# JADGardner/RENI

Measured on AMD Instinct MI355X. Metric: directional-samples/sec (fwd+bwd), 128x256 equirect, ND=36 latent, higher is better.
Workload: dtype bf16

## Files before the change

reni_amd/csrc/reni_capi.inc:

```
#include <dlfcn.h>

#include <cmath>
#include <cstdarg>
#include <cstdio>
#include <cstdlib>
#include <atomic>
#include <cstring>
#include <mutex>
#include <new>
#include <string>
#include <vector>

#include "../../include/reni_hip.h"

struct reni_plan {
  reni_desc d;
  int F_in;
  int64_t n_params;
  int64_t n_first;
  unsigned p_off_w[reni::MAX_LAYERS + 2];
  unsigned p_off_b[reni::MAX_LAYERS + 2];
  int M_in, N_out;
  int64_t n_map_params;
  unsigned mw_off[reni::MAX_MAP_LAYERS + 1], mb_off[reni::MAX_MAP_LAYERS + 1];
// ... 115 lines not shown
  }
  if (l.nwg < 1) l.nwg = 1;
  size_t o = 0;
  for (int st = 0; st < 2; ++st) {
    const bool mine = st == stage;
    if (mine) l.o_idxc = o;
    o += al256((size_t)B * 8);
    if (mine) l.o_Zc = o;
    o += al256((size_t)B * p->d.ndims * 3 * 4);
    if (mine) l.o_A = o;
    o += al256((size_t)B * H * 8 * 4);
    if (mine) l.o_afrag = o;
    if (l.persist) o += al256((size_t)B * (H / 32) * 1024);
    if (mine) l.o_xconst = o;
    o += al256((size_t)B * p->F_in * 4);
  }
  size_t w = 0;
  for (int i = 1; i <= L; ++i) { l.fwd_off[i] = (unsigned)w; w += al1k((size_t)g.img_hid + g.bias_hid); }
  l.fwd_off[L + 1] = (unsigned)w; w += al1k((size_t)g.img_hf + g.bias_head);
  for (int i = 1; i <= L; ++i) { l.bwd_off[i] = (unsigned)w; w += al1k((size_t)g.img_hid); }
  l.bwd_off[L + 1] = (unsigned)w; w += al1k((size_t)g.img_hb);
  l.wimg_bytes = w;
  w += 8192;
  l.o_wimg = o; o += al256(w);
  l.o_skip = o; o += 256;
  l.o_img_loss = o; o += al256((size_t)B * 16 * 4);
  l.o_stats = o; o += al256((size_t)B * 16 * 4);
  if (backward) {
    l.stash_per_wg = (size_t)(L + 1) * g.stash_layer_bytes * ((l.persist && !l.pdw && !l.wide_train) ? 2 : 1);
    l.frag = (p->d.dtype == RENI_BF16 && H == 256 && L >= 1 && (film || (flags & RENI_NEED_DW))) ? 1 : 0;
    if (p->d.dtype == RENI_F32 && H == 256 && L >= 1 && !film && (flags & RENI_NEED_DW)) l.frag = 2;
    l.o_stash = o; o += al256(l.stash_per_wg * (l.frag ? (size_t)l.n_tiles : (size_t)l.nwg));
    l.dwp_per_wg = (flags & RENI_NEED_DW) ? (size_t)(p->n_params - p->n_first) : 0;
    l.pkmax = ((l.n_tiles + l.nwg - 1) / l.nwg + l.tpi - 1) / l.tpi + 1;
    const size_t run_slots = (film && l.persist && !l.wide_train) ? (size_t)l.pkmax : 1;
    l.o_dwp = o; o += al256(l.dwp_per_wg * 4 * l.nwg * run_slots);
    l.o_dA_part = o; if (!l.pdw) o += al256((size_t)l.n_tiles * H * 8 * 4);
    l.o_tflag = l.o_tlist = l.o_tcount = l.o_imgcos = o;
    if (!film && !(flags & RENI_NEED_DW)) {
      l.o_tflag = o; o += al256((size_t)l.n_tiles * 4);
      l.o_tlist = o; o += al256((size_t)2 * l.n_tiles * 4);
      l.o_tcount = o; o += 256;
      l.o_imgcos = o; o += al256((size_t)B * 4);
      l.o_pcnt = o; o += al256((size_t)l.n_tiles * 4);
      l.o_pscan = o; o += al256((size_t)(l.n_tiles + 1) * 4);
      l.o_nlive = o; o += al256((size_t)B * 4);
      l.o_plist = o; o += al256((size_t)B * P * 4);
    }
    l.o_loss_part = o; o += al256((size_t)l.n_tiles * 4 * 16 * 4);
    l.o_dA = o; o += al256((size_t)B * H * 8 * 4);
    l.o_dw1p = o; if (l.pdw && (flags & RENI_NEED_DW)) o += al256((size_t)2 * l.nwg * run_slots * ((size_t)H * H + H) * 4);
    l.o_g1 = o; if (l.pdw) o += al256((size_t)((l.n_tiles + l.nwg - 1) / l.nwg) * l.nwg * (H / 16) * 4096);
    l.o_pruns = o; if (l.pdw) o += al256((size_t)l.nwg * l.pkmax * (H * 8 + 16) * 4);
    l.o_prunimg = o; if (l.pdw) o += al256((size_t)l.nwg * l.pkmax * (film ? 3 : 1) * 4);
    l.rt_chunk = reni::RT_CHUNK;
    l.nch = (l.tpi + l.rt_chunk - 1) / l.rt_chunk;
    l.o_part2 = o; o += al256((size_t)B * l.nch * (H * 8 + 16) * 4);
    l.o_mcol = o; o += al256((size_t)B * p->F_in * 4);
    l.o_ucol = o; o += al256((size_t)B * p->d.ndims * 3 * 4);
    l.o_dfp = o; if (film && !l.persist) o += al256((size_t)l.n_tiles * L * 2 * H * 4);
    const bool can = p->d.dtype == RENI_BF16 && L >= 1;
    l.stream = can && (H == 128 || H == 256) && (!l.persist || l.wide_train) && (film || (flags & RENI_NEED_DW)) ? 1 : 0;
    l.o_dws = o;
    l.o_dfr = o;
    l.o_runimg = o;
    if (l.frag == 2) o += al256((size_t)L * l.n_tiles * g.stash_layer_bytes);
// ... 98 lines not shown
bool dw1_ring_plan_ok(const reni_plan* p, int64_t P) { return !p->dw1_old && p->d.conditioning != RENI_COND_FILM && P % 128 == 0; }
bool dw1_ring_call_ok(const reni::MainArgs& a) { return (((uintptr_t)a.D | (uintptr_t)(a.d_bstride * 4)) & 15) == 0; }
int dw1_slots(bool ring, int nwg) { return ring ? nwg : 2 * nwg; }
bool l0x_rows_ok(const float* base, long long s0, long long s1, long long s2) {
  if (((uintptr_t)base | (uintptr_t)(s0 * 4)) & 15) return false;
  if (s1 == 3 && s2 == 1) return true;
  return s1 == 1 && ((uintptr_t)(s2 * 4) & 15) == 0;
}
bool l0x_plan_ok(const reni_plan* p, const Layout& l, int64_t P, uint32_t flags) {
  const int L = p->d.hidden_layers;
  return l.pdw && !p->no_l0x && dw1_ring_plan_ok(p, P) && spec_head(flags & RENI_NEED_DW, p->d.last_layer_linear, p->d.output_activation) &&
         L >= 3 && (L & 1) == 1;
}
bool l0x_call_ok(const reni::MainArgs& a) {
  return dw1_ring_call_ok(a) && train_spec(a, false) && l0x_rows_ok(a.target, a.ts0, a.ts1, a.ts2) && l0x_rows_ok(a.weight, a.ws0, a.ws1, a.ws2);
}
bool side_stream_plan_ok(const reni_plan* p, const Layout& l) { return l.pdw && !p->no_side_stream; }

int launch_dw1(const reni::MainArgs& a, int nwg, bool ring, hipStream_t s, bool l0x = false) {
#ifdef RENI_TRACE_DW1
  constexpr int TRACE = 8192;
#else
  constexpr int TRACE = 0;
#endif
  if (l0x)
    return timed_launch(reni::k_reni_l0_ring<128>, nwg, reni::L0Ring::THREADS, reni::L0Ring::LDS_BYTES + TRACE, s, a, PROF_DW1);
  if (a.film != nullptr) return timed_launch(s, PROF_DW1, "k_reni_dw1 (FiLM)", [&] { return reni::launch_dw1_film(a, 2 * nwg, s); });
  if (ring)
    return timed_launch(reni::k_reni_dw1_ring<128>, nwg, reni::Dw1Ring::THREADS, reni::Dw1Ring::LDS_BYTES + TRACE, s, a, PROF_DW1);
  return timed_launch(reni::k_reni_dw1<128>, 2 * nwg, 256, 2 * reni::TS_BYTES + TRACE, s, a, PROF_DW1);
}

int reduce_partials(const float* part, size_t per_wg, int nslot, float* out, int lo, int hi, const int* valid, const reni::LayerScale& lsc,
                    hipStream_t s) {
  RENI_LAUNCH(reni::k_reduce_partials, dim3((unsigned)((hi - lo + 63) / 64)), dim3(256), 0, s, part, per_wg, nslot, out, lo, hi, valid, lsc);
  return RENI_OK;
}

struct SideStream { hipStream_t s; hipEvent_t ev[3]; bool ok; };
std::mutex g_side_mu;
SideStream* side_stream() {
  static SideStream tab[16];
  static std::mutex mu;
  int dev = 0;
  if (hipGetDevice(&dev) != hipSuccess || dev < 0 || dev >= 16) return nullptr;
  std::lock_guard<std::mutex> lk(mu);
  SideStream& t = tab[dev];
  if (!t.ok) {
    if (hipStreamCreateWithFlags(&t.s, hipStreamNonBlocking) != hipSuccess) return nullptr;
    for (int i = 0; i < 3; ++i)
      if (hipEventCreateWithFlags(&t.ev[i], hipEventDisableTiming) != hipSuccess) return nullptr;
    t.ok = true;
  }
  return &t;
}

int launch_main(const reni_plan* p, int mode, const reni::MainArgs& a, int nwg, hipStream_t s) {
  const int H = p->d.hidden_features;
  const bool film = p->d.conditioning == RENI_COND_FILM, f32 = p->d.dtype == RENI_F32;
  return timed_launch(s, mode == reni::MODE_FWD_BWD ? PROF_FWD_BWD : mode == reni::MODE_STATS ? PROF_STATS : PROF_FWD, "fused kernel", [&] {
    if (f32) return film ? reni::launch_film_f32(H, mode, a, nwg, s) : reni::launch_main_f32(H, mode, a, nwg, s);
    return film ? reni::launch_film_bf16(H, mode, a, nwg, s) : reni::launch_main_bf16(H, mode, a, nwg, s);
  });
}

struct DeviceGuard {
  int prev = -1;
// ... 214 lines not shown
  uint32_t* state;
};

constexpr int LOSS_DOUT = 2;
struct BwdCall {
  int64_t B = 0, P = 0;
  const float *Z = nullptr, *D = nullptr, *params = nullptr;
  int64_t dbs = 0;
  const float *target = nullptr, *weight = nullptr, *dout = nullptr;
  const int64_t *ts = nullptr, *wst = nullptr;
  int loss_kind = RENI_LOSS_MSE;
  float alpha = 0.f, beta = 0.f;
  uint32_t flags = 0;
  float *out = nullptr, *loss_terms = nullptr, *dZ = nullptr, *dparams = nullptr;
  void* ws = nullptr;
  size_t ws_bytes = 0;
  void* stream = nullptr;
  const FilmIO* fio = nullptr;
  const int64_t* idx = nullptr;
  int64_t n_rows = 0;
  const StepFuse* fuse = nullptr;
  const WeightLists* lists = nullptr;
};

struct BwdPath {
  bool staged;
  int stage;
  bool use_cos;
  bool sparse;
  bool compact;
  bool cos_const;
  bool dw1_ring;
  bool l0x;
  bool fork;
  bool early_rest;
  bool dp_early;
  bool fused_tail;
  bool fuse_on;
  bool fpers;
  bool red2;
  int n_rest;
  int n_l1;
  bool rp_in_tail;
  bool ev_rest_done;
  bool dp_early_done;
};

struct Bwd {
  const reni_plan* p;
  const BwdCall& c;
  GeoRt g; Layout l; reni::MainArgs a;
  char* ws;
  hipStream_t s, se;
  const float* Z;
  int stage_in;
  float *img_loss, *stats, *dA, *part2;
  ListDst ld;
  reni::LayerScale lsc;
  BwdPath path;
};

bool call_uses_cos(const BwdCall& c) { return c.loss_kind == RENI_LOSS_TEST && c.beta != 0.f; }

BwdPath bwd_path(const reni_plan* p, const Layout& l, const BwdCall& c, const reni::MainArgs& a, int stage_in) {
  BwdPath t{};
  const int H = p->d.hidden_features, L = p->d.hidden_layers;
  const bool need_dw = (c.flags & RENI_NEED_DW) != 0;
  t.staged = stage_in >= 0;
  t.stage = t.staged ? stage_in : 0;
  t.n_rest = (int)(p->n_params - p->n_first);
  t.n_l1 = H * H + H;
  t.use_cos = call_uses_cos(c);
  t.sparse = (c.flags & (RENI_WEIGHT_SPARSE | RENI_WEIGHT_COMPACT)) && !c.fio && !need_dw && c.loss_kind != LOSS_DOUT &&
             c.weight != nullptr && c.out == nullptr;
  t.compact = t.sparse && (c.flags & RENI_WEIGHT_COMPACT);
  t.cos_const = t.sparse && c.lists && (c.lists->flags & RENI_WEIGHT_COS_CONSTANT);
  t.dw1_ring = dw1_ring_plan_ok(p, c.P) && dw1_ring_call_ok(a);
  t.l0x = l0x_plan_ok(p, l, c.P, c.flags) && l0x_call_ok(a);
  t.fork = side_stream_plan_ok(p, l) && !t.l0x && (c.fio || l.n_tiles >= 8 * l.nwg);
  t.early_rest = l.pdw && !c.fio && need_dw && L >= 1 && t.n_rest > t.n_l1;
  t.dp_early = c.fuse && c.fuse->comm && c.fuse->overlap;
  t.fused_tail = l.pdw && !c.fio;
  t.fuse_on = c.fuse && !c.fuse->comm && t.fused_tail && need_dw && (c.flags & RENI_NEED_DZ) && L >= 1;
  t.fpers = l.persist && !l.wide_train;
  t.red2 = L > 0 && t.fpers && need_dw;
  return t;
}

int bwd_validate(Bwd& x) {
  const reni_plan* p = x.p; const BwdCall& c = x.c;
  if (const int rc = c.fio ? check_film(p, c.fio, true) : RENI_OK) return rc;
  if (!c.fio && p && p->d.conditioning != RENI_COND_CONCAT) return fail(RENI_EINVAL, "FiLM plan: use the reni_film_* entry points");
  if (const int rc = check_common(p, c.B, c.P, c.fio ? c.fio->A : c.Z, c.D, c.params, c.ws)) return rc;
  if ((c.flags & RENI_NEED_DW) && !c.dparams) return fail(RENI_EINVAL, "RENI_NEED_DW set but dparams is NULL");
  if (!c.fio && (c.flags & RENI_NEED_DZ) && !c.dZ) return fail(RENI_EINVAL, "RENI_NEED_DZ set but dZ is NULL");
  if (c.loss_kind == LOSS_DOUT) {
    if (!c.dout) return fail(RENI_EINVAL, "dout is NULL");
  } else {
    if (c.loss_kind != RENI_LOSS_MSE && c.loss_kind != RENI_LOSS_TEST) return fail(RENI_EINVAL, "unknown loss_kind %d", c.loss_kind);
    if (!c.target || !c.weight || !c.ts || !c.wst) return fail(RENI_EINVAL, "target/weight (and their strides) must be non-NULL");
    if (!c.loss_terms) return fail(RENI_EINVAL, "loss_terms is NULL");
  }
  if (!geo_for(p, &x.g)) return fail(RENI_EUNSUPPORTED, "hidden_features=%d unsupported", p->d.hidden_features);
  return RENI_OK;
}

int bwd_layout(Bwd& x) {
  const BwdCall& c = x.c;
  const bool staged = c.fuse && (*c.fuse->state & 1u);
  x.stage_in = staged ? (int)((*c.fuse->state >> 1) & 1u) : -1;
  x.l = make_layout(x.p, x.g, c.B, c.P, c.flags, true, true, staged ? x.stage_in : 0);
// ... 59 lines not shown
}

int bwd_stats_pass(Bwd& x) {
  const BwdCall& c = x.c; const Layout& l = x.l;
  if (!x.path.use_cos || x.path.cos_const) return RENI_OK;
  reni::MainArgs st = x.a;
  st.out = nullptr; st.loss_kind = 0;
  if (x.path.sparse) { st.tlist = x.a.tlist + l.n_tiles; st.tcount = x.a.tcount + 1; }
  if (const int rc = l.persist ? launch_train(x.p, st, l.nwg, x.s, true) : launch_main(x.p, reni::MODE_STATS, st, l.nwg, x.s)) return rc;
  RENI_LAUNCH(reni::k_stats_image, dim3((unsigned)c.B), dim3(256), 0, x.s, (const float*)x.a.loss_part, l.tpi, c.weight, (long long)c.wst[0],
                     (long long)c.wst[2], c.beta, x.img_loss, x.stats, (const int*)x.ld.imgcos);
  return RENI_OK;
}

struct SideJoin {
  SideStream* side = nullptr;
  hipStream_t s = nullptr;
  ~SideJoin() { if (side && hipEventRecord(side->ev[2], side->s) == hipSuccess) (void)hipStreamWaitEvent(s, side->ev[2], 0); }
};

int bwd_fork_dw1(Bwd& x, std::unique_lock<std::mutex>& side_lock, SideJoin& side_join) {
  const reni_plan* p = x.p; const BwdCall& c = x.c; const Layout& l = x.l; BwdPath& path = x.path; hipStream_t s = x.s;
  if (!l.pdw) return RENI_OK;
  SideStream* side = path.fork ? side_stream() : nullptr;
  if (side) {
    side_lock.lock();
    HIP_TRY(hipEventRecord(side->ev[0], s));
    HIP_TRY(hipStreamWaitEvent(side->s, side->ev[0], 0));
    x.se = side->s;
    side_join.side = side; side_join.s = s;
  }
  path.rp_in_tail = path.early_rest && !side && !g_ev_rest && !path.dp_early;
  if (path.early_rest && !path.rp_in_tail) {
    int rc = reduce_partials(x.a.dwp, l.dwp_per_wg, l.nwg, c.dparams + p->n_first, path.n_l1, path.n_rest, nullptr, x.lsc, s);
    if (rc) return rc;
    if (g_ev_rest) { HIP_TRY(hipEventRecord(g_ev_rest, s)); path.ev_rest_done = true; }
    if (path.dp_early) {
      SideStream* cs = side_stream();
      if (!cs) return fail(RENI_EHIP, "no communication stream");
      if (!side_lock.owns_lock()) side_lock.lock();
      HIP_TRY(hipEventRecord(cs->ev[1], s));
      HIP_TRY(hipStreamWaitEvent(cs->s, cs->ev[1], 0));
      rc = rccl_allreduce_inplace(c.fuse->comm, c.dparams + p->n_first + path.n_l1, (size_t)(path.n_rest - path.n_l1), cs->s);
      if (rc) return rc;
      if (!side_join.side) { side_join.side = cs; side_join.s = s; }
      path.dp_early_done = true;
    }
  }
  return launch_dw1(x.a, l.nwg, path.dw1_ring, s, path.l0x);
}

int bwd_dw_consumers(Bwd& x) {
  const Layout& l = x.l; const reni::MainArgs& a = x.a; hipStream_t s = x.s;
  const int H = x.p->d.hidden_features;
  if (l.frag == 2) {
    const int lds = 4 * ((reni::Geo<reni::PolF32, 256>::T_BYTES + 1023) & ~1023);
    if (const int rc = timed_launch(reni::k_dw_frag32<256>, l.nwg, 256, lds, s, a, PROF_DWS)) return rc;
  }
  if (l.wide_train && (x.c.flags & RENI_NEED_DW)) {
    if (const int rc = timed_launch(s, PROF_DWS, "k_wide_head_dw", [&] { return reni::launch_wide_head_dw(a, l.nwg, s); })) return rc;
  }
  if (l.stream) {
    static_assert(reni::Geo<reni::PolBF16, 256>::T_BYTES_AL == 36864 && reni::Geo<reni::PolBF16, 128>::T_BYTES_AL == 34816,
                  "stream record sizes (make_layout)");
    const bool film = x.c.fio != nullptr;
    void (*fn)(const reni::MainArgs) = nullptr;
    if (H == 256) fn = film ? reni::k_dw_frag<256, true> : reni::k_dw_frag<256, false>;
// ... 57 lines not shown
  const reni_plan* p = x.p; const BwdCall& c = x.c; const Layout& l = x.l; const BwdPath& path = x.path; const reni::MainArgs& a = x.a;
  hipStream_t s = x.s, se = x.se;
  const int H = p->d.hidden_features;
  const bool need_dw = (c.flags & RENI_NEED_DW) != 0;
  reni::TailArgs t;
  t.dA = x.dA; t.W0 = c.params; t.Z = x.Z; t.xconst = (const float*)(x.ws + l.o_xconst);
  t.mcol = (float*)(x.ws + l.o_mcol); t.ucol = (float*)(x.ws + l.o_ucol);
  t.dZ = c.dZ; t.dW0 = c.dparams; t.db0 = c.dparams ? c.dparams + (size_t)H * p->F_in : nullptr;
  t.alpha2 = (c.loss_kind == RENI_LOSS_TEST) ? c.alpha : 0.f;
  t.eq = p->d.equivariance; t.nd = p->d.ndims; t.F_in = p->F_in; t.H = H; t.B = (int)c.B;
  if (!path.fuse_on && need_dw && l.pdw && p->d.hidden_layers >= 1) {
    if (const int rc = reduce_partials(a.dw1p, (size_t)path.n_l1, dw1_slots(path.dw1_ring, l.nwg), c.dparams + p->n_first, 0, path.n_l1, nullptr, x.lsc, s)) return rc;
  }
  reni::TailFusedArgs f;
  memset(&f, 0, sizeof(f));
  f.t = t;
  f.img_loss = x.img_loss; f.stats = x.stats; f.P = (int)c.P; f.nz = (int)(c.B * p->d.ndims * 3); f.has_cos = path.use_cos ? 1 : 0;
  f.has_prior = (c.loss_kind == RENI_LOSS_TEST) ? 1 : 0; f.alpha = c.alpha; f.beta = c.beta;
  f.loss_terms = (c.loss_kind != LOSS_DOUT) ? c.loss_terms : nullptr;
  f.need_dz = (c.flags & RENI_NEED_DZ) ? 1 : 0;
  f.need_dw0 = need_dw ? 1 : 0;
  f.dw0_gx = (p->F_in + 1 + 255) / 256;
  f.idx_now = path.staged ? (const long long*)c.idx : nullptr;
  f.idx_staged = path.staged ? (const long long*)(x.ws + l.o_idxc) : nullptr;
  f.skip_flag = c.fuse ? (int*)(x.ws + l.o_skip) : nullptr;
  const unsigned nb = (unsigned)((f.need_dz ? c.B : 0) + 1 + (f.need_dw0 ? f.dw0_gx * H : 0));
  if (path.fused_tail) {
    f.pruns = a.pruns; f.prun_image = a.prun_image; f.nwg = l.nwg; f.kmax = l.pkmax; f.tpi = l.tpi; f.n_tiles = l.n_tiles;
    f.dA_out = x.dA;
    const unsigned ny = f.need_dz ? (unsigned)((p->F_in + 63) / 64) : 1u;
    unsigned gx = (unsigned)c.B;
    if (path.rp_in_tail) {
      f.rp_part = a.dwp; f.rp_per_wg = l.dwp_per_wg; f.rp_nwg = l.nwg; f.rp_out = c.dparams + p->n_first; f.rp_lo = path.n_l1; f.rp_n = path.n_rest; f.rp_ls = x.lsc;
      gx += ((unsigned)((path.n_rest - path.n_l1 + 63) / 64) + ny - 1) / ny;
    }
    RENI_LAUNCH(reni::k_tail_a, dim3(gx, ny), dim3(256), (size_t)reni::tail_a_lds_bytes(H), se, f);
  } else if (c.flags & RENI_NEED_DZ) {
    RENI_LAUNCH(reni::k_tail_m, dim3((unsigned)c.B, (unsigned)((p->F_in + 63) / 64)), dim3(256), 0, se, t);
  }
  RENI_LAUNCH(reni::k_tail_b, dim3(nb), dim3(256), 0, se, f);
  if (need_dw && !path.fused_tail && path.n_rest > 0) {
    if (const int rc = reduce_partials(a.dwp, l.dwp_per_wg, l.nwg, c.dparams + p->n_first, 0, path.n_rest, nullptr, x.lsc, s)) return rc;
  }
  if (g_ev_rest && !path.ev_rest_done) HIP_TRY(hipEventRecord(g_ev_rest, s));
  return RENI_OK;
}

int bwd_fused_step(Bwd& x, SideJoin& side_join) {
  const reni_plan* p = x.p; const BwdCall& c = x.c; const Layout& l = x.l; const BwdPath& path = x.path; hipStream_t s = x.s;
  const StepFuse& fu = *c.fuse;
  if (side_join.side) {
    HIP_TRY(hipEventRecord(side_join.side->ev[2], side_join.side->s));
    HIP_TRY(hipStreamWaitEvent(s, side_join.side->ev[2], 0));
    side_join.side = nullptr;
  }
  if (fu.comm) {
    const size_t n_early = path.dp_early_done ? (size_t)(path.n_rest - path.n_l1) : 0;
    EvPair ev;
    const bool timed = prof_begin(s, &ev, PROF_COMM);
    int rc = rccl_allreduce_max_i32(fu.comm, (int*)(x.ws + l.o_skip), 1, s);
    if (rc) return rc;
    rc = rccl_allreduce_inplace(fu.comm, c.dparams, (size_t)p->n_params - n_early, s);
    if (rc) return rc;
    if (timed) HIP_TRY(hipEventRecord(ev.b, s));
  }
  reni::Adam2Args ad;
  ad.p = fu.params; ad.g = c.dparams; ad.m = fu.m_dec; ad.v = fu.v_dec; ad.n = p->n_params;
// ... 914 lines not shown
```

reni_amd/csrc/reni_dev_common.inc:

```


DEV constexpr int rowmap(int r, int hi) { return (r & 3) + 8 * (r >> 2) + 4 * hi; }

struct PolF32 {
  static constexpr bool BF = false;
  static constexpr int FRAGB = 4;
  static constexpr int KF = 2;
  static constexpr int TS = 2;
  static constexpr int WPS = 1;
  static constexpr int HEAD_BWD_KS = 3;
  static constexpr int STASH_CH_PER_RB = 4;
  using Frag = float;
  static DEV f32x16 mfma(Frag a, Frag b, f32x16 c) {
    return __builtin_amdgcn_mfma_f32_32x32x2f32(a, b, c, 0, 0, 0);
  }
  static DEV void drain() {
    __builtin_amdgcn_sched_barrier(0);
    asm volatile("s_nop 15\n\ts_nop 3");
    __builtin_amdgcn_sched_barrier(0);
  }
};
struct PolBF16 {
  static constexpr bool BF = true;
  static constexpr int FRAGB = 16;
// ... 458 lines not shown
          } else {
            *p = first ? acc[m][r] : (*p + acc[m][r]);
          }
        } else if constexpr (KIND == DW_HEAD) {
          if (j < 3) {
            float* p = dst_w + (size_t)j * ldw + row;
            *p = first ? acc[m][r] : (*p + acc[m][r]);
          }
        } else {
          const float lo = __shfl_down(acc[m][r], 8, 64);
          if (j < 8) dst_w[(size_t)row * 8 + j] = acc[m][r] + ((j < 4) ? lo : 0.f);
        }
      }
    }
  }
  if constexpr (!DO_B) {
    return;
  } else if constexpr (KIND == DW_HIDDEN) {
    dbacc += __shfl_xor(dbacc, 32, 64);
    if (wave < NBR && wave < NBLK && hi == 0) {
      if (rscale != nullptr) dbacc *= rscale[32 * (wave % NBR) + j];
      float* p = dst_b + 32 * (wave % NBR) + j;
      *p = first ? dbacc : (*p + dbacc);
    }
  } else if constexpr (KIND == DW_HEAD) {
    dbacc += __shfl_xor(dbacc, 32, 64);
    if (wave == 0 && hi == 0 && j < 3) {
      float* p = dst_b + j;
      *p = first ? dbacc : (*p + dbacc);
    }
  }
}

struct FilmDw {
  const float* fl;
  float* fs;
  const float* W;
  const float* b;
  float* out;
  int do_w;
};

DEV float half_sum(float t) {
#pragma unroll
  for (int o = 16; o >= 1; o >>= 1) t += __shfl_xor(t, o, 64);
  return t;
}

template <class Pol, int H, int NBR, int NBC, int KIND, bool FILM = false>
DEV void dw_phase(char* TA, char* TB, const float (&rows)[NBR][16], const float (&cols)[NBC][16],
                  float* dst_w, float* dst_b, int ldw, bool first, int wave, int lane, int dbg = 0,
                  const FilmDw* fd = nullptr) {
  constexpr int MYB = (NBR * NBC + 3) / 4;
  constexpr int NBLK = NBR * NBC;
  constexpr int NROUND = 4 / Geo<Pol, H>::ROUND_WAVES;
  const int hi = lane >> 5, j = lane & 31;
  const int tid = wave * 64 + lane;
  if constexpr (MYB <= 4) {
    f32x16 acc[MYB];
    acc_zero<MYB>(acc);
    float dbacc = 0.f;
#pragma unroll 1
    for (int round = 0; round < NROUND; ++round) {
      __syncthreads();
      if (wave / Geo<Pol, H>::ROUND_WAVES == round && !(dbg & 4)) {
        t_write<Pol, H, NBR>(TA, rows, wave % Geo<Pol, H>::ROUND_WAVES, hi, j);
// ... 177 lines not shown
```

reni_amd/csrc/reni_dev_small.inc:

```

DEV void reduce_film_runs_body(const MainArgs& a, int H, int nruns, float* dfilm, const int bx, const int by) {
  const float* dfr = a.dfr;
  const int* run_image = a.run_image;
  const int L = a.L;
  const float* params = a.params;
  const unsigned n_first = a.n_first;
  const unsigned* p_off_b = a.p_off_b;
  const int b = bx, i = by * 256 + threadIdx.x;
  const bool live = i < L * H;
  const int l = live ? i / H : 0, f = i - l * H;
  __shared__ int vl[1024];
  __shared__ int nv;
  float s0 = 0.f, s1 = 0.f;
  for (int base = 0; base < nruns; base += 1024) {
    const int cnt = nruns - base < 1024 ? nruns - base : 1024;
    __syncthreads();
    if (threadIdx.x < 64) {
      int c = 0;
      for (int w0 = 0; w0 < cnt; w0 += 64) {
        const int w = w0 + (int)threadIdx.x;
        const bool ok = w < cnt && run_image[base + w] == b;
        const unsigned long long m = __ballot(ok);
        if (ok) vl[c + __popcll(m & ((1ull << threadIdx.x) - 1ull))] = base + w;
        c += __popcll(m);
// ... 388 lines not shown
  const int i = (int)blockIdx.x;
  if (i < a.n_prep && a.film_A != nullptr) afrag_from_A_body(a.film_A, a.film_afrag, a.film_scale, a.prep.H, a.film_B, i);
  else if (i < a.n_prep) prep_image_body(a.prep, i / a.prep_gy, i % a.prep_gy, smem);
  else pack_body<Pol>(ka, (i - a.n_prep) % a.pack_gx, (i - a.n_prep) / a.pack_gx, a.pack_gx);
}
template __global__ void k_prologue<PolF32>(const PrologueArgs, const PackArgs);
template __global__ void k_prologue<PolBF16>(const PrologueArgs, const PackArgs);

struct LayerScale { int n_hid, L; float c[MAX_LAYERS + 1]; };
DEV float layer_scale(const LayerScale& ls, int e) {
  int k = ls.n_hid > 0 ? e / ls.n_hid : 0;
  k = k < ls.L ? k : ls.L;
  return ls.c[k];
}
DEV void reduce_partials_body(const float* part, size_t per_wg, int nwg, float* dparams, int lo, int n, int blk, float (*red2)[64],
                              const LayerScale& ls) {
  const int lane = threadIdx.x & 63, grp = threadIdx.x >> 6;
  const int e = lo + blk * 64 + lane;
  float s[8];
#pragma unroll
  for (int q = 0; q < 8; ++q) s[q] = 0.f;
  if (e < n) {
    int q = grp;
    for (; q + 28 < nwg; q += 32) {
#pragma unroll
      for (int u = 0; u < 8; ++u) s[u] += part[(size_t)(q + 4 * u) * per_wg + e];
    }
    for (; q < nwg; q += 4) s[0] += part[(size_t)q * per_wg + e];
  }
  red2[grp][lane] = ((s[0] + s[1]) + (s[2] + s[3])) + ((s[4] + s[5]) + (s[6] + s[7]));
  __syncthreads();
  if (grp == 0 && e < n) dparams[e] = ((red2[0][lane] + red2[1][lane]) + (red2[2][lane] + red2[3][lane])) * layer_scale(ls, e);
}
DEV void reduce_partials_valid_body(const float* part, size_t per_wg, int nwg, float* dparams, int lo, int n, const int* valid, int blk) {
  __shared__ int vl[2048];
  __shared__ int nv;
  __shared__ float red[4][64];
  const int lane = threadIdx.x & 63, grp = threadIdx.x >> 6;
  const int e = lo + blk * 64 + lane;
  float s[8];
#pragma unroll
  for (int q = 0; q < 8; ++q) s[q] = 0.f;
  for (int base = 0; base < nwg; base += 2048) {
    const int cnt = nwg - base < 2048 ? nwg - base : 2048;
    __syncthreads();
    if (threadIdx.x < 64) {
      int c = 0;
      for (int w0 = 0; w0 < cnt; w0 += 64) {
        const int w = w0 + (int)threadIdx.x;
        const bool ok = w < cnt && valid[base + w] >= 0;
        const unsigned long long m = __ballot(ok);
        if (ok) vl[c + __popcll(m & ((1ull << threadIdx.x) - 1ull))] = base + w;
        c += __popcll(m);
      }
      if (threadIdx.x == 0) nv = c;
    }
    __syncthreads();
    if (e < n) {
      const int m = nv;
      int q = grp;
      for (; q + 28 < m; q += 32) {
#pragma unroll
        for (int u = 0; u < 8; ++u) s[u] += part[(size_t)vl[q + 4 * u] * per_wg + e];
      }
      for (; q < m; q += 4) s[0] += part[(size_t)vl[q] * per_wg + e];
    }
  }
  red[grp][lane] = ((s[0] + s[1]) + (s[2] + s[3])) + ((s[4] + s[5]) + (s[6] + s[7]));
  __syncthreads();
  if (grp == 0 && e < n) dparams[e] = (red[0][lane] + red[1][lane]) + (red[2][lane] + red[3][lane]);
}
__global__ void __launch_bounds__(256) k_reduce_partials(const float* part, size_t per_wg, int nwg,
                                                          float* dparams, int lo, int n, const int* valid, const LayerScale ls) {
  const int i = lo + blockIdx.x * 256 + threadIdx.x;
  if (valid != nullptr) {
    reduce_partials_valid_body(part, per_wg, nwg, dparams, lo, n, valid, (int)blockIdx.x);
    return;
  }
  (void)i;
  __shared__ float red2[4][64];
  reduce_partials_body(part, per_wg, nwg, dparams, lo, n, (int)blockIdx.x, red2, ls);
}

struct FilmReduce2 { int H, nruns, B, gy; float* dfilm; const float* part; size_t per_wg; int nslot; float* dparams; int n; const int* valid; };
__global__ void __launch_bounds__(256) k_film_reduce2(const MainArgs a, const FilmReduce2 r) {
  const int i = (int)blockIdx.x, nb1 = r.B * r.gy;
  if (i < nb1) reduce_film_runs_body(a, r.H, r.nruns, r.dfilm, i / r.gy, i % r.gy);
  else reduce_partials_valid_body(r.part, r.per_wg, r.nslot, r.dparams, 0, r.n, r.valid, i - nb1);
}

constexpr int RT_CHUNK = 4;
__global__ void __launch_bounds__(256) k_reduce_tiles_a(const float* dA_part, const float* loss_part,
                                                        int tiles_per_image, int H, float* part2, int have_dA, int chunk,
                                                        const int* tflag = nullptr) {
  const int b = blockIdx.x, ch = blockIdx.y, nch = gridDim.y;
  const int t0 = ch * chunk, t1 = min(t0 + chunk, tiles_per_image);
  float* out = part2 + ((size_t)b * nch + ch) * (H * 8 + 16);
  if (have_dA) {
    const int k = threadIdx.x & 7;
    constexpr int MAXQ = 8;
    const int nq = (H * 8 + 255) / 256;
    float s[MAXQ];
#pragma unroll
    for (int q = 0; q < MAXQ; ++q) s[q] = 0.f;
    if (k < 5) {
#pragma unroll 4
      for (int t = t0; t < t1; ++t) {
        if (tflag != nullptr && tflag[b * tiles_per_image + t] == 0) continue;
        const float* row = dA_part + (size_t)(b * tiles_per_image + t) * H * 8 + threadIdx.x;
#pragma unroll
        for (int q = 0; q < MAXQ; ++q)
          if (q < nq && q * 256 + (int)threadIdx.x < H * 8) s[q] += row[q * 256];
      }
    }
// ... 371 lines not shown
  const float* m = a.mcol + (size_t)b * F;
  const float* u = a.ucol + (size_t)b * nd * 3;
  const float* z = a.Z + (size_t)b * nd * 3;
  for (int t = tid; t < nd * 3; t += 256) {
    const int i = t / 3, k = t - 3 * i;
    float val = 0.f;
    if (a.eq == 1) {
      if (k == 1) {
        val = m[nd + nd * nd + 1 + i];
      } else {
        val = u[i * 3 + k];
        for (int q = 0; q < nd; ++q) val += (m[nd + i * nd + q] + m[nd + q * nd + i]) * z[q * 3 + k];
      }
    } else if (a.eq == 2) {
      val = u[i * 3 + k];
      for (int q = 0; q < nd; ++q) val += (m[nd + i * nd + q] + m[nd + q * nd + i]) * z[q * 3 + k];
    } else {
      val = u[i * 3 + k] + m[nd + i * 3 + k];
    }
    val += 2.f * a.alpha2 * z[t];
    a.dZ[(size_t)b * nd * 3 + t] = val;
  }
}

struct TailFusedArgs {
  TailArgs t;
  const float* pruns; const int* prun_image; int nwg, kmax, tpi, n_tiles;
  float* dA_out; float* img_loss;
  const float* stats; int P, nz, has_cos, has_prior; float alpha, beta; float* loss_terms;
  int need_dz, need_dw0, dw0_gx;
  const long long* idx_now; const long long* idx_staged;
  int* skip_flag;
  const float* rp_part; size_t rp_per_wg; int rp_nwg, rp_lo, rp_n; float* rp_out; LayerScale rp_ls;
};
constexpr int TF_LMAX = 512;
constexpr int tail_a_lds_bytes(int H) { return (H * 8 + 16) * 4 + 4 * 64 * 4 * 4 + TF_LMAX * 4; }
__global__ void __launch_bounds__(256) k_tail_a(const TailFusedArgs a) {
  extern __shared__ __attribute__((aligned(16))) char smem[];
  if ((int)blockIdx.x >= a.t.B) {
    const int blk = ((int)blockIdx.x - a.t.B) * (int)gridDim.y + (int)blockIdx.y;
    reduce_partials_body(a.rp_part, a.rp_per_wg, a.rp_nwg, a.rp_out, a.rp_lo, a.rp_n, blk, (float (*)[64])smem, a.rp_ls);
    return;
  }
  const int H = a.t.H, F = a.t.F_in, nd = a.t.nd, b = blockIdx.x, tid = threadIdx.x;
  float* const dAs = (float*)smem;
  float (*const red)[64][4] = (float (*)[64][4])(dAs + H * 8 + 16);
  int* const list = (int*)(red + 4);
  __shared__ int nlist;
  const int c = tid & 63, rg = tid >> 6;
  const int col = blockIdx.y * 64 + c;
  constexpr int RPT = 32;
  const int h0 = rg * (H / 4), h1 = h0 + H / 4;
  float w[RPT];
  if (a.need_dz) {
#pragma unroll
    for (int u = 0; u < RPT; ++u) w[u] = (col < F && h0 + u < h1) ? a.t.W0[(size_t)(h0 + u) * F + col] : 0.f;
  }
  int g0 = (int)((long long)b * a.tpi * a.nwg / a.n_tiles) - 1;
  int g1 = (int)((long long)(b + 1) * a.tpi * a.nwg / a.n_tiles) + 1;
  g0 = g0 < 0 ? 0 : g0;
  g1 = g1 > a.nwg - 1 ? a.nwg - 1 : g1;
  const int ncand = (g1 - g0 + 1) * a.kmax;
  if (tid < 64) {
    int n = 0;
    for (int c0 = 0; c0 < ncand; c0 += 64) {
      const int cc = c0 + tid;
      const bool ok = cc < ncand && a.prun_image[g0 * a.kmax + cc] == b;
      const unsigned long long m = __ballot(ok);
      const int pos = n + __popcll(m & ((1ull << tid) - 1ull));
      if (ok && pos < TF_LMAX) list[pos] = g0 * a.kmax + cc;
      n += __popcll(m);
    }
    if (tid == 0) nlist = n;
// ... 274 lines not shown
```

reni_amd/csrc/reni_dev_train.inc:

```

constexpr int TAIL_RB2 = 1, TAIL_DWDX = 1, TAIL_DWDX_A = 1;
#ifdef RENI_TU_TRAIN_FILM
constexpr int TAIL_RB1 = 5;
#else
constexpr int TAIL_RB1 = 3;
#endif
template <int N, class F>
DEV void static_for_down(F&& f) {
  if constexpr (N >= 1) {
    f(std::integral_constant<int, N>{});
    static_for_down<N - 1>(f);
  }
}

template <int I, int N, class F>
DEV void static_for_up(F&& f) {
  if constexpr (I < N) {
    f(std::integral_constant<int, I>{});
    static_for_up<I + 1, N>(f);
  }
}

template <int H>
struct GeoP {
// ... 213 lines not shown
}

template <int H, bool DW, bool STATS = false, bool FILM = false, bool SPEC = false, bool L0X = false>
__global__ void __launch_bounds__(DW ? 256 : 512, 1) k_reni_train_bf16(const MainArgs a) {
  static_assert(!(DW && STATS), "the statistics instance has no backward pass");
  static_assert(!SPEC || DW, "SPEC is an instance of the training kernel");
  static_assert(!L0X || (SPEC && !FILM), "L0X is a form of the concat SPEC instance");
  static_assert(!FILM || DW || STATS, "FiLM: the training instance serves the frozen decoder too");
  using Pol = PolBF16;
  using G = Geo<Pol, H>;
  using GP = GeoP<H>;
  static_assert(H == 128, "sample-major transposition image is laid out for H = 128");
  constexpr int NRB = G::NRB, NKS = G::NKS;
  constexpr int MYB_H = (NRB * NRB + 3) / 4;
  constexpr int PMAX = 5;
  extern __shared__ __attribute__((aligned(1024))) char smem[];
  char* const TA = smem + 2 * GP::WBSZ;
  char* const TB = TA + GP::TSZ;
  float* const hdw = (float*)(TB + GP::TSZ);
  char* const HF = TB + GP::TSZ + 2048;
  char* const HB = HF + GP::HFSZ;
  float* const dAacc = (float*)(HB + GP::HBSZ);
  constexpr int FT_FLOATS = (PMAX + 1) * 2 * H;
  float* const ftab_base = FILM ? (DW ? dAacc + H * 8 : (float*)TB) : nullptr;

#ifdef RENI_TRACE
  unsigned long long* const trace_lds = (unsigned long long*)(smem + GP::LDS_BYTES + GP::LACC_BYTES);
  int trace_n = 0;
#ifndef RENI_TRACE_WAVE
#define RENI_TRACE_WAVE 0
#endif
  const bool trace_on = a.trace != nullptr && blockIdx.x == 0 && __builtin_amdgcn_readfirstlane(threadIdx.x >> 6) == RENI_TRACE_WAVE;
#define TRACE(tag) do { __builtin_amdgcn_sched_barrier(0); if (trace_on && trace_n < 500) { trace_lds[trace_n] = ((unsigned long long)__builtin_amdgcn_s_memtime() & 0xffffffffffffull) | ((unsigned long long)(tag) << 48); ++trace_n; } __builtin_amdgcn_sched_barrier(0); } while (0)
#else
#define TRACE(tag) do {} while (0)
#endif
  const int tid = threadIdx.x;
  constexpr int NW = DW ? 4 : 8, NHALF = NW / 4, DG = DW ? DMA_GROUPS : 2;
  const int wave = __builtin_amdgcn_readfirstlane(tid >> 6);
  const int wq = wave & 3, half = wave >> 2;
  const int lane = tid & 63, hi = lane >> 5, j = lane & 31;
  char* const stash = a.stash + (size_t)blockIdx.x * (G::STASH_LAYER_BYTES * (DW ? 1 : 2));
  const size_t stash_layer_stride = (size_t)gridDim.x * (G::STASH_LAYER_BYTES * (DW ? 1 : 2));
  float* const dwp = a.dwp + (size_t)blockIdx.x * a.dwp_per_wg;
  const int L = a.L;
  const int nstep = L0X ? 2 * L + 1 : 2 * L + 2;
  int wpar_v = 0;

  static_assert(MYB_H == 4, "sixteen AGPR tiles = 4 layers x 4 column blocks");
  if constexpr (DW) agpr_zero_seq(std::make_integer_sequence<int, 256>{});
  float pdb[PMAX];
#pragma unroll
  for (int l = 0; l < PMAX; ++l) pdb[l] = 0.f;
  if constexpr (DW) {
    for (int i = tid; i < 3 * H + 32; i += 256) hdw[i] = 0.f;
    for (int i = tid; i < H * 8; i += 256) dAacc[i] = 0.f;
  }
  constexpr bool LACC = SPEC;
  f32x4* const lacc = (f32x4*)(dAacc + H * 8 + (FILM ? FT_FLOATS : 0));
  float* const hdb = hdw + 3 * H + 16;
  float* const loss_run = hdw + 3 * H + 8;
  if constexpr (DW) { if (tid < 4) loss_run[tid] = 0.f; }
  if constexpr (LACC) { if (tid < 128) lacc[tid] = f32x4{0.f, 0.f, 0.f, 0.f}; }
  const int act = SPEC ? 1 : a.act;
  const bool last_linear = SPEC ? true : (a.last_linear != 0);
  const int loss_kind = SPEC ? 0 : a.loss_kind;
  float* const out_img = SPEC ? nullptr : a.out;
  const float inv3p = 1.0f / (3.0f * (float)a.P);
// ... 864 lines not shown
              float dbs = pdb[l - 1];
              dbs += __shfl_xor(dbs, 32, 64);
#pragma unroll
              for (int r = 0; r < 16; ++r) {
                const int row = 32 * wave + rowmap(r, hio);
                float pr = 0.f;
#pragma unroll
                for (int m = 0; m < MYB_H; ++m) pr = __builtin_fmaf(Wl[(unsigned)(row * H + 32 * m + jo)], t[m][r], pr);
                pr = half_sum(pr);
                const float fq = tq[row] * 6.283185307179586f;
                if (jo == r) fr[(unsigned)((l - 1) * 2 * H + row)] = (fq != 0.f) ? pr / fq : 0.f;
              }
              if (hio == 0) {
                const int row = 32 * wave + jo;
                const float fq = tq[row] * 6.283185307179586f;
                fr[(unsigned)((l - 1) * 2 * H + H + row)] = (fq != 0.f) ? dbs / fq : 0.f;
              }
              if (a.need_dw) dw_flush<Pol, H, NRB, NRB, DW_HIDDEN, MYB_H>(t, pdb[l - 1], dwr + a.p_off_w[l], dwr + a.p_off_b[l], H, true, wave, hio * 32 + jo);
              agpr_zero_range<64 * (l - 2)>(std::make_integer_sequence<int, 64>{});
              pdb[l - 1] = 0.f;
            }
          };
          film_flush(std::integral_constant<int, 2>{});
          film_flush(std::integral_constant<int, 3>{});
          film_flush(std::integral_constant<int, 4>{});
          film_flush(std::integral_constant<int, 5>{});
        }
        ++run_k;
      }
    }
    if constexpr (INCR) { cur_b = nxt_b; cur_tin = nxt_tin; }
    TRACE(9);
  }
#ifdef RENI_TRACE
  if (trace_on) {
    for (int i = lane; i < trace_n; i += 64) a.trace[i] = (long long)trace_lds[i];
  }
#endif
  int tid_e = L0X ? (int)((unsigned)tid16 >> 4) : tid;
  asm volatile("" : "+v"(tid_e));
  if constexpr (DW) {
    for (int k = run_k + tid_e; k < a.pkmax; k += 256) a.prun_image[blockIdx.x * a.pkmax + k] = -1;
  }
  if constexpr (DW && FILM) {
    if (a.need_dw) {
      if constexpr (LACC) {
        f32x4 v = f32x4{0.f, 0.f, 0.f, 0.f};
        if ((tid_e & 63) < 32) v = lacc[(tid_e >> 6) * 32 + (tid_e & 31)];
        const float s0 = wave_sum(v[1]), s1 = wave_sum(v[2]), s2 = wave_sum(v[3]);
        if ((tid_e & 63) == 0) { float* o = hdb + 4 * (tid_e >> 6); o[0] = s0; o[1] = s1; o[2] = s2; }
      }
      __syncthreads();
      float* const dw0 = a.dwp + (size_t)blockIdx.x * a.pkmax * a.dwp_per_wg;
      for (int i = tid_e; i < 3 * H; i += 256) dw0[a.p_off_w[L + 1] + i] = hdw[i];
      if (tid_e < 3) dw0[a.p_off_b[L + 1] + tid_e] = (hdb[tid_e] + hdb[4 + tid_e]) + (hdb[8 + tid_e] + hdb[12 + tid_e]);
    }
  } else if constexpr (DW) {
    if constexpr (LACC) {
      f32x4 v = f32x4{0.f, 0.f, 0.f, 0.f};
      if ((tid_e & 63) < 32) v = lacc[(tid_e >> 6) * 32 + (tid_e & 31)];
      const float s0 = wave_sum(v[1]), s1 = wave_sum(v[2]), s2 = wave_sum(v[3]);
      if ((tid_e & 63) == 0) { float* o = hdb + 4 * (tid_e >> 6); o[0] = s0; o[1] = s1; o[2] = s2; }
    }
    __syncthreads();
    for (int i = tid_e; i < 3 * H; i += 256) dwp[a.p_off_w[L + 1] + i] = hdw[i];
    if (tid_e < 3) dwp[a.p_off_b[L + 1] + tid_e] = (hdb[tid_e] + hdb[4 + tid_e]) + (hdb[8 + tid_e] + hdb[12 + tid_e]);
    asm volatile("s_nop 15\n\ts_nop 15" ::: "memory");
    auto flush_layer = [&](auto lc) {
      constexpr int l = decltype(lc)::value;
      if (l <= L) {
        f32x16 t[MYB_H] = {agpr_read_tile<4 * (l - 2) + 0>(), agpr_read_tile<4 * (l - 2) + 1>(),
                           agpr_read_tile<4 * (l - 2) + 2>(), agpr_read_tile<4 * (l - 2) + 3>()};
        dw_flush<Pol, H, NRB, NRB, DW_HIDDEN, MYB_H>(t, pdb[l - 1], dwp + a.p_off_w[l], dwp + a.p_off_b[l], H, true, wave, L0X ? (tid_e & 63) : lane);
      }
    };
    flush_layer(std::integral_constant<int, 2>{});
    flush_layer(std::integral_constant<int, 3>{});
    flush_layer(std::integral_constant<int, 4>{});
    flush_layer(std::integral_constant<int, 5>{});
  }
}
#ifdef RENI_TU_CORE
template __global__ void k_reni_train_bf16<128, true>(const MainArgs);
template __global__ void k_reni_train_bf16<128, true, false, false, true>(const MainArgs);
template __global__ void k_reni_train_bf16<128, true, false, false, true, true>(const MainArgs);
template __global__ void k_reni_train_bf16<128, false>(const MainArgs);
template __global__ void k_reni_train_bf16<128, false, true>(const MainArgs);
#endif

#if defined(RENI_TRACE_DW1)
#define TRACE1(tag) do { __builtin_amdgcn_sched_barrier(0); if (trace_on && trace_n < 1000) { trace_lds[trace_n] = ((unsigned long long)__builtin_amdgcn_s_memtime() & 0xffffffffffffull) | ((unsigned long long)(tag) << 48); ++trace_n; } __builtin_amdgcn_sched_barrier(0); } while (0)
#else
#define TRACE1(tag) do {} while (0)
#endif
template <int H, bool FILM = false>
__global__ void __launch_bounds__(256, 2) k_reni_dw1(const MainArgs a) {
  using Pol = PolBF16;
  using G = Geo<Pol, H>;
  constexpr int NRB = G::NRB, NKS = G::NKS;
  constexpr int MYB_H = (NRB * NRB + 3) / 4;
  extern __shared__ __attribute__((aligned(1024))) char smem[];
  char* const TA = smem;
  char* const TB = smem + TS_BYTES;
  const int tid = threadIdx.x;
  const int wave = __builtin_amdgcn_readfirstlane(tid >> 6);
  const int lane = tid & 63, hi = lane >> 5, j = lane & 31;
#if defined(RENI_TRACE_DW1)
  unsigned long long* const trace_lds = (unsigned long long*)(smem + 2 * TS_BYTES);
  int trace_n = 0;
  const bool trace_on = a.trace != nullptr && blockIdx.x == 0 && wave == 0;
#endif
  TRACE1(100);
#if defined(RENI_TRACE_DW1) && RENI_TRACE_DW1 == 2
// ... 373 lines not shown
```

Baseline: 1.324 billion.

## Write hidden-layer dW partials in quad-row layout and reduce with vector loads

On the l0x path, the train kernel now flushes hidden-layer weight-gradient partials in a quad-row interleaved layout, writing four consecutive rows as one 16-byte store per lane instead of scattered scalar stores. A new quad reduction kernel, also usable inside the fused tail, sums these partials with f32x4 loads and several loads in flight, then remaps each word back to the flat parameter index. Per-workgroup slots are padded to 64 floats to keep them aligned. This adds layout coupling between the producer kernel and the reducer, plus some index arithmetic, and it moves the trace flush to the end of the kernel.

```diff
diff --git a/reni_amd/csrc/reni_capi.inc b/reni_amd/csrc/reni_capi.inc
--- a/reni_amd/csrc/reni_capi.inc
+++ b/reni_amd/csrc/reni_capi.inc
@@ -171,6 +171,7 @@
     if (p->d.dtype == RENI_F32 && H == 256 && L >= 1 && !film && (flags & RENI_NEED_DW)) l.frag = 2;
     l.o_stash = o; o += al256(l.stash_per_wg * (l.frag ? (size_t)l.n_tiles : (size_t)l.nwg));
     l.dwp_per_wg = (flags & RENI_NEED_DW) ? (size_t)(p->n_params - p->n_first) : 0;
+    if (l.pdw) l.dwp_per_wg = (l.dwp_per_wg + 63) & ~(size_t)63;
     l.pkmax = ((l.n_tiles + l.nwg - 1) / l.nwg + l.tpi - 1) / l.tpi + 1;
     const size_t run_slots = (film && l.persist && !l.wide_train) ? (size_t)l.pkmax : 1;
     l.o_dwp = o; o += al256(l.dwp_per_wg * 4 * l.nwg * run_slots);
@@ -335,7 +336,12 @@
 }
 
 int reduce_partials(const float* part, size_t per_wg, int nslot, float* out, int lo, int hi, const int* valid, const reni::LayerScale& lsc,
-                    hipStream_t s) {
+                    hipStream_t s, int quad_H = 0) {
+  if (quad_H > 0) {
+    if (valid != nullptr || (per_wg & 3) || (lo & 3) || ((uintptr_t)part & 15)) return fail(RENI_EINVAL, "internal: quad-row partials need untagged, 16-byte aligned slots");
+    RENI_LAUNCH(reni::k_reduce_partials_quad, dim3((unsigned)((hi - lo + reni::QUAD_BLK_WORDS - 1) / reni::QUAD_BLK_WORDS)), dim3(256), 0, s, part, per_wg, nslot, out, lo, hi, quad_H, lsc);
+    return RENI_OK;
+  }
   RENI_LAUNCH(reni::k_reduce_partials, dim3((unsigned)((hi - lo + 63) / 64)), dim3(256), 0, s, part, per_wg, nslot, out, lo, hi, valid, lsc);
   return RENI_OK;
 }
@@ -616,6 +622,7 @@
   bool cos_const;
   bool dw1_ring;
   bool l0x;
+  bool part_quad;
   bool fork;
   bool early_rest;
   bool dp_early;
@@ -661,6 +668,7 @@
   t.cos_const = t.sparse && c.lists && (c.lists->flags & RENI_WEIGHT_COS_CONSTANT);
   t.dw1_ring = dw1_ring_plan_ok(p, c.P) && dw1_ring_call_ok(a);
   t.l0x = l0x_plan_ok(p, l, c.P, c.flags) && l0x_call_ok(a);
+  t.part_quad = t.l0x;
   t.fork = side_stream_plan_ok(p, l) && !t.l0x && (c.fio || l.n_tiles >= 8 * l.nwg);
   t.early_rest = l.pdw && !c.fio && need_dw && L >= 1 && t.n_rest > t.n_l1;
   t.dp_early = c.fuse && c.fuse->comm && c.fuse->overlap;
@@ -786,7 +794,7 @@
   }
   path.rp_in_tail = path.early_rest && !side && !g_ev_rest && !path.dp_early;
   if (path.early_rest && !path.rp_in_tail) {
-    int rc = reduce_partials(x.a.dwp, l.dwp_per_wg, l.nwg, c.dparams + p->n_first, path.n_l1, path.n_rest, nullptr, x.lsc, s);
+    int rc = reduce_partials(x.a.dwp, l.dwp_per_wg, l.nwg, c.dparams + p->n_first, path.n_l1, path.n_rest, nullptr, x.lsc, s, path.part_quad ? p->d.hidden_features : 0);
     if (rc) return rc;
     if (g_ev_rest) { HIP_TRY(hipEventRecord(g_ev_rest, s)); path.ev_rest_done = true; }
     if (path.dp_early) {
@@ -910,7 +918,10 @@
     unsigned gx = (unsigned)c.B;
     if (path.rp_in_tail) {
       f.rp_part = a.dwp; f.rp_per_wg = l.dwp_per_wg; f.rp_nwg = l.nwg; f.rp_out = c.dparams + p->n_first; f.rp_lo = path.n_l1; f.rp_n = path.n_rest; f.rp_ls = x.lsc;
-      gx += ((unsigned)((path.n_rest - path.n_l1 + 63) / 64) + ny - 1) / ny;
+      f.rp_quad = path.part_quad ? 1 : 0;
+      if (f.rp_quad && ((l.dwp_per_wg | (size_t)path.n_l1) & 3)) return fail(RENI_EINVAL, "internal: quad-row partials need 16-byte aligned slots");
+      const int per_blk = f.rp_quad ? reni::QUAD_BLK_WORDS : 64;
+      gx += ((unsigned)((path.n_rest - path.n_l1 + per_blk - 1) / per_blk) + ny - 1) / ny;
     }
     RENI_LAUNCH(reni::k_tail_a, dim3(gx, ny), dim3(256), (size_t)reni::tail_a_lds_bytes(H), se, f);
   } else if (c.flags & RENI_NEED_DZ) {
diff --git a/reni_amd/csrc/reni_dev_common.inc b/reni_amd/csrc/reni_dev_common.inc
--- a/reni_amd/csrc/reni_dev_common.inc
+++ b/reni_amd/csrc/reni_dev_common.inc
@@ -514,6 +514,23 @@
   }
 }
 
+DEV constexpr unsigned quad_word(int row, int col, int H) { return (unsigned)((((row >> 2) * H + col) << 2) + (row & 3)); }
+template <int H, int NBR, int MYB>
+DEV void dw_flush_quad(const f32x16 (&acc)[MYB], float dbacc, float* dst_w, float* dst_b, int wave, int lane) {
+  static_assert(NBR == 4 && MYB == H / 32, "pinned form: wave w owns row block w and every column block");
+  static_assert(rowmap(4, 0) == 8 && rowmap(3, 1) == 7, "registers 4 i .. 4 i + 3: rows 8 i + 4 hi .. + 3 of the block");
+  const int hi = lane >> 5, j = lane & 31;
+  float* const base = dst_w + ((size_t)((8 * wave + hi) * H + j) << 2);
+#pragma unroll
+  for (int m = 0; m < MYB; ++m) {
+#pragma unroll
+    for (int i = 0; i < 4; ++i)
+      *(f32x4*)(base + ((2 * i * H + 32 * m) << 2)) = f32x4{acc[m][4 * i], acc[m][4 * i + 1], acc[m][4 * i + 2], acc[m][4 * i + 3]};
+  }
+  dbacc += __shfl_xor(dbacc, 32, 64);
+  if (hi == 0) dst_b[32 * wave + j] = dbacc;
+}
+
 struct FilmDw {
   const float* fl;
   float* fs;
diff --git a/reni_amd/csrc/reni_dev_small.inc b/reni_amd/csrc/reni_dev_small.inc
--- a/reni_amd/csrc/reni_dev_small.inc
+++ b/reni_amd/csrc/reni_dev_small.inc
@@ -444,6 +444,52 @@
   __syncthreads();
   if (grp == 0 && e < n) dparams[e] = ((red2[0][lane] + red2[1][lane]) + (red2[2][lane] + red2[3][lane])) * layer_scale(ls, e);
 }
+DEV int quad_word_to_flat(int w, int H, int n_hid, int L) {
+  const int k = w / n_hid, t = w - k * n_hid;
+  if (k >= L || t >= H * H) return w;
+  const int q = t >> 2, rq = q / H, col = q - rq * H;
+  return k * n_hid + (4 * rq + (t & 3)) * H + col;
+}
+constexpr int QUAD_BLK_WORDS = 64;
+template <class Emit>
+DEV void reduce_partials_quad_body(const float* part, size_t per_wg, int nwg, int lo, int n, int blk, f32x4 (*red4)[64], int H, int n_hid, int L,
+                                   Emit&& emit) {
+  const int lane = threadIdx.x & 63, grp = threadIdx.x >> 6;
+  const int l16 = lane & 15, uq = lane >> 4;
+  const int w = lo + blk * QUAD_BLK_WORDS + 4 * l16;
+  f32x4 s0 = f32x4{0.f, 0.f, 0.f, 0.f}, s1 = s0;
+  if (w < n) {
+    const float* const p = part + w + (size_t)(8 * uq) * per_wg;
+    int q = grp;
+    for (; q + 124 < nwg; q += 128) {
+      f32x4 v[8];
+#pragma unroll
+      for (int k = 0; k < 4; ++k) {
+        v[2 * k] = *(const f32x4*)(p + (size_t)(q + 32 * k) * per_wg);
+        v[2 * k + 1] = *(const f32x4*)(p + (size_t)(q + 32 * k + 4) * per_wg);
+      }
+      __builtin_amdgcn_sched_barrier(0);
+#pragma unroll
+      for (int k = 0; k < 4; ++k) { s0 += v[2 * k]; s1 += v[2 * k + 1]; }
+    }
+    for (; q + 28 < nwg; q += 32) {
+      const f32x4 a = *(const f32x4*)(p + (size_t)q * per_wg), b = *(const f32x4*)(p + (size_t)(q + 4) * per_wg);
+      s0 += a; s1 += b;
+    }
+    if (uq == 0) {
+      for (; q < nwg; q += 4) s0 += *(const f32x4*)(p + (size_t)q * per_wg);
+    }
+  }
+  red4[grp][lane] = s0 + s1;
+  __syncthreads();
+  if (threadIdx.x < QUAD_BLK_WORDS) {
+    const int m = (int)threadIdx.x >> 2, c = (int)threadIdx.x & 3, ww = lo + blk * QUAD_BLK_WORDS + (int)threadIdx.x;
+    float g[4];
+#pragma unroll
+    for (int gg = 0; gg < 4; ++gg) g[gg] = (red4[gg][m][c] + red4[gg][16 + m][c]) + (red4[gg][32 + m][c] + red4[gg][48 + m][c]);
+    if (ww < n) emit(quad_word_to_flat(ww, H, n_hid, L), (g[0] + g[1]) + (g[2] + g[3]));
+  }
+}
 DEV void reduce_partials_valid_body(const float* part, size_t per_wg, int nwg, float* dparams, int lo, int n, const int* valid, int blk) {
   __shared__ int vl[2048];
   __shared__ int nv;
@@ -492,6 +538,12 @@
   (void)i;
   __shared__ float red2[4][64];
   reduce_partials_body(part, per_wg, nwg, dparams, lo, n, (int)blockIdx.x, red2, ls);
+}
+__global__ void __launch_bounds__(256) k_reduce_partials_quad(const float* part, size_t per_wg, int nwg, float* dparams, int lo, int n, int H,
+                                                               const LayerScale ls) {
+  __shared__ f32x4 red4[4][64];
+  reduce_partials_quad_body(part, per_wg, nwg, lo, n, (int)blockIdx.x, red4, H, ls.n_hid, ls.L,
+                            [&](int e, float v) { dparams[e] = v * layer_scale(ls, e); });
 }
 
 struct FilmReduce2 { int H, nruns, B, gy; float* dfilm; const float* part; size_t per_wg; int nslot; float* dparams; int n; const int* valid; };
@@ -929,6 +981,7 @@
   const long long* idx_now; const long long* idx_staged;
   int* skip_flag;
   const float* rp_part; size_t rp_per_wg; int rp_nwg, rp_lo, rp_n; float* rp_out; LayerScale rp_ls;
+  int rp_quad;
 };
 constexpr int TF_LMAX = 512;
 constexpr int tail_a_lds_bytes(int H) { return (H * 8 + 16) * 4 + 4 * 64 * 4 * 4 + TF_LMAX * 4; }
@@ -936,6 +989,12 @@
   extern __shared__ __attribute__((aligned(16))) char smem[];
   if ((int)blockIdx.x >= a.t.B) {
     const int blk = ((int)blockIdx.x - a.t.B) * (int)gridDim.y + (int)blockIdx.y;
+    if (a.rp_quad) {
+      static_assert(tail_a_lds_bytes(32) >= 4 * 64 * 16, "red4 fits the dynamic LDS at every width");
+      reduce_partials_quad_body(a.rp_part, a.rp_per_wg, a.rp_nwg, a.rp_lo, a.rp_n, blk, (f32x4 (*)[64])smem, a.t.H, a.rp_ls.n_hid, a.rp_ls.L,
+                                [&](int e, float v) { a.rp_out[e] = v * layer_scale(a.rp_ls, e); });
+      return;
+    }
     reduce_partials_body(a.rp_part, a.rp_per_wg, a.rp_nwg, a.rp_out, a.rp_lo, a.rp_n, blk, (float (*)[64])smem, a.rp_ls);
     return;
   }
diff --git a/reni_amd/csrc/reni_dev_train.inc b/reni_amd/csrc/reni_dev_train.inc
--- a/reni_amd/csrc/reni_dev_train.inc
+++ b/reni_amd/csrc/reni_dev_train.inc
@@ -269,8 +269,10 @@
 #endif
   const bool trace_on = a.trace != nullptr && blockIdx.x == 0 && __builtin_amdgcn_readfirstlane(threadIdx.x >> 6) == RENI_TRACE_WAVE;
 #define TRACE(tag) do { __builtin_amdgcn_sched_barrier(0); if (trace_on && trace_n < 500) { trace_lds[trace_n] = ((unsigned long long)__builtin_amdgcn_s_memtime() & 0xffffffffffffull) | ((unsigned long long)(tag) << 48); ++trace_n; } __builtin_amdgcn_sched_barrier(0); } while (0)
+#define TRACE_FLUSH(slot, tag) do { __builtin_amdgcn_sched_barrier(0); if (trace_on) trace_lds[slot] = ((unsigned long long)__builtin_amdgcn_s_memtime() & 0xffffffffffffull) | ((unsigned long long)(tag) << 48); __builtin_amdgcn_sched_barrier(0); } while (0)
 #else
 #define TRACE(tag) do {} while (0)
+#define TRACE_FLUSH(slot, tag) do {} while (0)
 #endif
   const int tid = threadIdx.x;
   constexpr int NW = DW ? 4 : 8, NHALF = NW / 4, DG = DW ? DMA_GROUPS : 2;
@@ -1201,11 +1203,6 @@
     if constexpr (INCR) { cur_b = nxt_b; cur_tin = nxt_tin; }
     TRACE(9);
   }
-#ifdef RENI_TRACE
-  if (trace_on) {
-    for (int i = lane; i < trace_n; i += 64) a.trace[i] = (long long)trace_lds[i];
-  }
-#endif
   int tid_e = L0X ? (int)((unsigned)tid16 >> 4) : tid;
   asm volatile("" : "+v"(tid_e));
   if constexpr (DW) {
@@ -1235,12 +1232,14 @@
     for (int i = tid_e; i < 3 * H; i += 256) dwp[a.p_off_w[L + 1] + i] = hdw[i];
     if (tid_e < 3) dwp[a.p_off_b[L + 1] + tid_e] = (hdb[tid_e] + hdb[4 + tid_e]) + (hdb[8 + tid_e] + hdb[12 + tid_e]);
     asm volatile("s_nop 15\n\ts_nop 15" ::: "memory");
+    TRACE_FLUSH(510, 10);
     auto flush_layer = [&](auto lc) {
       constexpr int l = decltype(lc)::value;
       if (l <= L) {
         f32x16 t[MYB_H] = {agpr_read_tile<4 * (l - 2) + 0>(), agpr_read_tile<4 * (l - 2) + 1>(),
                            agpr_read_tile<4 * (l - 2) + 2>(), agpr_read_tile<4 * (l - 2) + 3>()};
-        dw_flush<Pol, H, NRB, NRB, DW_HIDDEN, MYB_H>(t, pdb[l - 1], dwp + a.p_off_w[l], dwp + a.p_off_b[l], H, true, wave, L0X ? (tid_e & 63) : lane);
+        if constexpr (L0X) dw_flush_quad<H, NRB, MYB_H>(t, pdb[l - 1], dwp + a.p_off_w[l], dwp + a.p_off_b[l], wave, tid_e & 63);
+        else dw_flush<Pol, H, NRB, NRB, DW_HIDDEN, MYB_H>(t, pdb[l - 1], dwp + a.p_off_w[l], dwp + a.p_off_b[l], H, true, wave, L0X ? (tid_e & 63) : lane);
       }
     };
     flush_layer(std::integral_constant<int, 2>{});
@@ -1248,6 +1247,15 @@
     flush_layer(std::integral_constant<int, 4>{});
     flush_layer(std::integral_constant<int, 5>{});
   }
+#ifdef RENI_TRACE
+  if constexpr (DW && !FILM) {
+    asm volatile("s_waitcnt vmcnt(0)" ::: "memory");
+    TRACE_FLUSH(511, 11);
+  }
+  if (trace_on) {
+    for (int i = (int)(threadIdx.x & 63); i < 512; i += 64) a.trace[i] = (i < trace_n || (DW && !FILM && i >= 510)) ? (long long)trace_lds[i] : 0ll;
+  }
+#endif
 }
 #ifdef RENI_TU_CORE
 template __global__ void k_reni_train_bf16<128, true>(const MainArgs);
```

After: 1.358 billion, median of 6. +2.6%, better.
